# mobinasri/flagger

Measured on AMD Instinct MI355X. Metric: coverage windows/sec through EM+decode; achieved HBM GB/s vs roofline, higher is better.
Workload: dtype f64

## Files before the change

### flagger_amd/csrc/hf_create.h

```cpp
#pragma once

namespace {
struct PinnedArena {
    char *a = nullptr, *b = nullptr, *c = nullptr; std::thread th;
    ~PinnedArena() { if (th.joinable()) th.join(); pin_cache().release(a); pin_cache().release(b); pin_cache().release(c); }
};

struct KeyMarks {
    size_t words = 0;
    uint64_t gen = 0;
    std::atomic<int> claimed{0};
    std::vector<std::vector<uint16_t>> tabs;
    KeyMarks() : tabs(HF_PARTS + 8) {}
    uint16_t* mine() {
        static thread_local uint64_t tl_gen = 0;
        static thread_local int tl_slot = -1;
        if (tl_gen != gen) {
            tl_slot = claimed.fetch_add(1);
            tl_gen = gen;
            if (tl_slot < (int) tabs.size()) tabs[(size_t) tl_slot].assign(words, 0);
        }
        return tl_slot < (int) tabs.size() ? tabs[(size_t) tl_slot].data() : nullptr;
    }
};
// ... 382 lines not shown
        if (cw.ctrace) std::fprintf(stderr, "[hf_create] %d emission keys, %d (key, transition class) rows, %d slow windows\n",
                                    ctx->n_keys, n_combo, ctx->n_slow);
    }
    std::vector<SegDesc>& segs = ctx->h_segs;
    std::vector<int32_t>& cseg0 = cw.cseg0;
    cseg0.assign(C + 1, 0);
    int64_t nslots = 0;
    for (size_t c = 0; c < C; c++) {
        const int64_t t0 = w->chunk_off[c], T = w->chunk_off[c + 1] - t0;
        cseg0[c] = (int32_t) segs.size();
        if (T <= 0) continue;
        const int64_t nsg = (T + SMAX - 1) / SMAX, sz = (T + nsg - 1) / nsg;
        const int first = (int) segs.size();
        for (int64_t k = 0; k * sz < T; k++) {
            SegDesc d;
            std::memset(&d, 0, sizeof d);
            const int64_t w0 = k * sz, n = T - w0 < sz ? T - w0 : sz;
            d.t0 = t0 + w0; d.n = (int) n; d.L = (int) ((n + NL - 1) / NL);
            d.slot0 = (int32_t) nslots; nslots += (int64_t) d.L * NL;
            d.chunk_slow0 = ctx->n_combo + cw.soff[c];
            d.seg0 = first; d.k = (int) k; d.chunk = (int) c; d.ident_row = ctx->n_arows;
            d.reg_first = (int32_t) ((w->annot[t0] & 0xFC00000000000000ULL) >> 58);
            d.reg_last = (int32_t) ((w->annot[t0 + T - 1] & 0xFC00000000000000ULL) >> 58);
            segs.push_back(d);
        }
        const int nsc = (int) segs.size() - first;
        const int32_t spare = (int32_t) nslots++;
        for (int k = 0; k < nsc; k++) {
            segs[(size_t) (first + k)].nseg = nsc;
            segs[(size_t) (first + k)].next_slot = k + 1 < nsc ? segs[(size_t) (first + k + 1)].slot0 : spare;
        }
    }
    cseg0[C] = (int32_t) segs.size();
    ctx->h_cseg0 = cseg0;
    if (nslots < INT32_MAX) {
        ctx->nseg = (int) segs.size(); ctx->n_slots = nslots;
        CTRY(dev_upload(ctx, cw.stg, &ctx->d_chunk_seg0, cseg0.data(), cseg0.size()));
        CALLOC(ctx->d_seg_ready, segs.size() * 4);
        hipMemsetAsync(ctx->d_seg_ready, 0, segs.size() * 4, nullptr);
        CALLOC(ctx->d_seg_ll, segs.size() * 8);
        CALLOC(ctx->d_Pseg, segs.size() * 16 * 8);
    } else segs.clear();
    cw.phase("segments");
    return HF_OK;
}

struct StatsPlan {
    bool compact = false, planned = false;
    int64_t n_pos = 0;
    size_t np = 0;
    std::vector<int32_t> cnt;
    std::vector<int32_t> g_pos0;
    std::vector<int32_t> grp_ar, grp_n, grp_off;
    std::vector<RowSlot> rslots; std::vector<int32_t> rwreg, rwoff;
    std::vector<int64_t> extra0;
    std::vector<int32_t> h_spare;
};
int64_t plan_place_extras(CreateWork& cw, StatsPlan& pl, size_t sp, int64_t from, bool with_first_two) {
    hf_ctx* ctx = cw.ctx; const hf_windows* w = cw.w;
    int64_t p = from;
    const auto& sb = ctx->subs[sp];
    for (int c = sb.c0; c < sb.c1; c++) {
        const int64_t T = w->chunk_off[c + 1] - w->chunk_off[c];
        pl.extra0[(size_t) c] = p;
        p += T <= 0 ? 0 : (with_first_two ? (T < 2 ? T : 2) : 0) + 1;
        pl.extra0[(size_t) c + 1] = p;
    }
    for (int k = sb.seg0; k < sb.seg1; k++) ctx->h_segs[(size_t) k].trash_pos = (int32_t) p++;
    return p;
}

void plan_groups_and_slots(CreateWork& cw, StatsPlan& pl, int bpw) {
    hf_ctx* ctx = cw.ctx; const hf_windows* w = cw.w;
    const int n_regions = cw.n_regions;
    const size_t n_ar = cw.h_arow_src.size(), S = (size_t) cw.n_sub;
    const bool compact = pl.compact;
    std::vector<hf_ctx::SubPass>& subs = ctx->subs;
    struct Occ { int32_t region, ar; };
    std::vector<Occ> occ;
    const size_t MMr = (size_t) ctx->M * ctx->M;
    for (size_t r = 0; r < n_ar; r++) {
        bool any = false;
        for (size_t sp = 0; sp < S && !any; sp++) any = pl.cnt[sp * n_ar + r] != 0;
        if (!any) continue;
        const int64_t er = cw.h_arow_src[r];
        int32_t reg;
        if (er < ctx->n_lut) reg = (int32_t) ((size_t) er / MMr);
        else reg = (int32_t) ((w->annot[(size_t) cw.slow[(size_t) (er - ctx->n_lut)]] & 0xFC00000000000000ULL) >> 58);
        occ.push_back({reg, (int32_t) r});
    }
    if (n_regions > 1) std::stable_sort(occ.begin(), occ.end(), [](const Occ& a, const Occ& b) { return a.region < b.region; });
    const size_t nocc = occ.size();
    pl.g_pos0.assign(S * n_ar, 0);
    const size_t unit = (size_t) 16 * (size_t) bpw;
    struct RowBase { int32_t g0, slot0, go; int64_t p0; };
    std::vector<RowBase> rb(S * nocc, RowBase{0, 0, 0, 0});
    size_t n_grp = 0, n_slot = 0;
    int64_t next_pos = 0;
    for (size_t sp = 0; sp < S; sp++) {
        subs[sp].g0 = (int) n_grp; subs[sp].p0 = next_pos;
        for (size_t oi = 0; oi < nocc; oi++) {
            const size_t r = (size_t) occ[oi].ar;
            const int32_t c_ = pl.cnt[sp * n_ar + r];
            if (!c_) continue;
            RowBase& B = rb[sp * nocc + oi];
            B.g0 = (int32_t) n_grp;
            B.p0 = compact ? next_pos : subs[sp].p0 + (int64_t) (n_grp - (size_t) subs[sp].g0) * HF_GRP_PAIRS;
            n_grp += (size_t) ((c_ + HF_GRP_PAIRS - 1) / HF_GRP_PAIRS);
            if (compact) next_pos += c_;
        }
        if (!compact) next_pos = subs[sp].p0 + (int64_t) (n_grp - (size_t) subs[sp].g0) * HF_GRP_PAIRS;
        subs[sp].g1 = (int) n_grp;
        next_pos = plan_place_extras(cw, pl, sp, next_pos, true);
        subs[sp].p1 = next_pos;
    }
    pl.n_pos = next_pos;
    {
        size_t oi0 = 0;
        for (int reg = 0; reg < n_regions; reg++) {
            pl.rwoff[(size_t) reg] = (int32_t) (n_slot / unit);
            size_t oi1 = oi0;
            while (oi1 < nocc && occ[oi1].region == reg) oi1++;
            for (size_t sp = 0; sp < S; sp++) {
                int64_t open_row = -1; size_t run_slot0 = n_slot; int32_t run_groups = 0;
                for (size_t oi = oi0; oi < oi1; oi++) {
                    const size_t r = (size_t) occ[oi].ar;
                    const int32_t c_ = pl.cnt[sp * n_ar + r];
                    if (!c_) continue;
                    const int64_t er = cw.h_arow_src[r];
                    const int32_t ng = (c_ + HF_GRP_PAIRS - 1) / HF_GRP_PAIRS;
                    if (er != open_row) { n_slot = run_slot0 + (size_t) ((run_groups + HF_ROWSLOT_GROUPS - 1) / HF_ROWSLOT_GROUPS); run_slot0 = n_slot; run_groups = 0; open_row = er; }
                    rb[sp * nocc + oi].slot0 = (int32_t) run_slot0; rb[sp * nocc + oi].go = run_groups;
                    run_groups += ng;
                }
                n_slot = run_slot0 + (size_t) ((run_groups + HF_ROWSLOT_GROUPS - 1) / HF_ROWSLOT_GROUPS);
            }
            n_slot = (n_slot + HF_RS_WPB * unit - 1) / (HF_RS_WPB * unit) * (HF_RS_WPB * unit);
            for (size_t k = (size_t) pl.rwoff[(size_t) reg]; k < n_slot / unit; k++) pl.rwreg.push_back(reg);
            oi0 = oi1;
        }
    }
    pl.grp_ar.assign((n_grp + 3) / 4 * 4, 0); pl.grp_n.assign((n_grp + 3) / 4 * 4, 0);
    pl.grp_off.assign(n_grp + 1, 0);
    pl.rslots.assign(n_slot, RowSlot{-1, 0, 0, 0});
    for (size_t sp = 0; sp < S; sp++)
        for (size_t oi = 0; oi < nocc; oi++) {
            const size_t r = (size_t) occ[oi].ar;
            const int32_t c_ = pl.cnt[sp * n_ar + r];
            if (!c_) continue;
            const int64_t er = cw.h_arow_src[r];
            const RowBase B = rb[sp * nocc + oi];
            pl.g_pos0[sp * n_ar + r] = (int32_t) B.p0;
            int32_t xpx;
            if (er < ctx->n_lut) xpx = (int32_t) (((size_t) er / (size_t) ctx->M) % (size_t) ctx->M) | ((int32_t) ((size_t) er % (size_t) ctx->M) << 8);
            else { const size_t t = (size_t) cw.slow[(size_t) (er - ctx->n_lut)]; xpx = (int32_t) (w->cov[t] & 0xffu) | ((int32_t) (w->cov[t - 1] & 0xffu) << 8); }
            int64_t p = B.p0;
            for (int32_t j = 0, left = c_; left > 0; j++, left -= HF_GRP_PAIRS) {
                const size_t g = (size_t) (B.g0 + j);
                const int32_t here = left < HF_GRP_PAIRS ? left : HF_GRP_PAIRS;
                pl.grp_ar[g] = (int32_t) r; pl.grp_n[g] = here; pl.grp_off[g] = (int32_t) p;
                p += compact ? here : HF_GRP_PAIRS;
                RowSlot& sl = pl.rslots[(size_t) B.slot0 + (size_t) ((B.go + j) / HF_ROWSLOT_GROUPS)];
                if ((B.go + j) % HF_ROWSLOT_GROUPS == 0) { sl.row = (int32_t) er; sl.g0 = (int32_t) g; sl.ng = 1; sl.xpx = xpx; }
                else sl.ng++;
            }
        }
    pl.rwoff[(size_t) n_regions] = (int32_t) (pl.rslots.size() / unit);
    ctx->n_parts = 1;
    for (int reg = 0; reg < n_regions; reg++) if (pl.rwoff[(size_t) reg + 1] > pl.rwoff[(size_t) reg]) ctx->n_parts++;
    ctx->n_groups = (int) n_grp;
    pl.grp_off[n_grp] = (int32_t) (n_grp ? pl.grp_off[n_grp - 1] + (compact ? pl.grp_n[n_grp - 1] : HF_GRP_PAIRS) : 0);
    ctx->plan_compact = compact;
    pl.planned = true;
}

int plan_upload(CreateWork& cw, StatsPlan& pl) {
    hf_ctx* ctx = cw.ctx;
    const int n_regions = cw.n_regions;
    const size_t C = cw.C;
    {
        std::vector<int32_t> boff((size_t) n_regions * 256 + 1, 0), blist;
        auto bin_of = [&](size_t k) {
            const int x = pl.rslots[k].xpx & 0xff;
            return (size_t) pl.rwreg[k / ((size_t) 16 * (size_t) ctx->rs_bpw)] * 256 + (size_t) (x < HF_NB_MAX_COVERAGE ? x : HF_NB_MAX_COVERAGE - 1);
        };
        for (size_t k = 0; k < pl.rslots.size(); k++) if (pl.rslots[k].row >= 0) boff[bin_of(k) + 1]++;
        for (size_t b = 0; b + 1 < boff.size(); b++) boff[b + 1] += boff[b];
        blist.resize((size_t) boff.back());
        std::vector<int32_t> fill(boff.begin(), boff.end() - 1);
        for (size_t k = 0; k < pl.rslots.size(); k++) if (pl.rslots[k].row >= 0) blist[(size_t) fill[bin_of(k)]++] = (int32_t) k;
        CTRY(dev_upload(ctx, cw.stg, &ctx->d_bin_off, boff.data(), boff.size()));
        CTRY(dev_upload(ctx, cw.stg, &ctx->d_bin_list, blist.data(), blist.size()));
        CALLOC(ctx->d_slot_h, pl.rslots.size() * 4 * 8);
        CALLOC(ctx->d_H, (size_t) n_regions * 4 * 256 * 8);
    }
    ctx->n_rowwaves = (int) (pl.rslots.size() / ((size_t) 16 * (size_t) ctx->rs_bpw));
    CTRY(dev_upload(ctx, cw.stg, &ctx->d_grp_ar, pl.grp_ar.data(), pl.grp_ar.size()));
    CTRY(dev_upload(ctx, cw.stg, &ctx->d_grp_n, pl.grp_n.data(), pl.grp_n.size()));
    if (pl.compact) CTRY(dev_upload(ctx, cw.stg, &ctx->d_grp_off, pl.grp_off.data(), pl.grp_off.size()));
    CTRY(dev_upload(ctx, cw.stg, &ctx->d_rowslots, pl.rslots.data(), pl.rslots.size()));
    CTRY(dev_upload(ctx, cw.stg, &ctx->d_rw_region, pl.rwreg.data(), pl.rwreg.size()));
    CTRY(dev_upload(ctx, cw.stg, &ctx->d_rw_off, pl.rwoff.data(), pl.rwoff.size()));
    ctx->h_rw_off = pl.rwoff;
    CALLOC(ctx->d_grp_sums, (size_t) pl.grp_ar.size() * 16 * 8);
    CALLOC(ctx->d_chunk_ll, C * 8);
    CALLOC(ctx->d_rw_stats, (size_t) ctx->n_rowwaves * (16 + 9 + 2 + 3 * 16 + 1) * 8);
    ctx->rows_ready = true;
    return HF_OK;
}

int create_statistics_plan(CreateWork& cw) {
    hf_ctx* ctx = cw.ctx; const hf_windows* w = cw.w;
    const size_t N = cw.N, C = cw.C;
    const int n_regions = cw.n_regions;
    if (!(N > 0 && C > 0 && ctx->nseg > 0)) return HF_OK;
    const size_t n_ar = cw.h_arow_src.size();
    const size_t S = (size_t) cw.n_sub;
    StatsPlan pl;
    pl.cnt.assign(S * n_ar + 1, 0);
    pl.rwoff.assign((size_t) n_regions + 1, 0);
    pl.extra0.assign(C + 1, 0);
    pl.h_spare.assign(C, 0);
    for (size_t c = 0; c < C; c++) {
        const int64_t T = w->chunk_off[c + 1] - w->chunk_off[c];
        pl.np += (size_t) (T > 2 ? T - 2 : 0);
    }
    for (auto& h : cw.pcnt)
        if (!h.empty())
            for (size_t r = 0; r < S * n_ar; r++) { const int32_t here = h[r]; h[r] = pl.cnt[r]; pl.cnt[r] += here; }
    int64_t n_groups_all = 0;
    for (size_t r = 0; r < S * n_ar; r++) n_groups_all += (pl.cnt[r] + HF_GRP_PAIRS - 1) / HF_GRP_PAIRS;
    const bool dense = n_groups_all * HF_GRP_PAIRS <= 4 * (int64_t) pl.np + (4 << 20);
    pl.compact = !dense;
    const char* const force = std::getenv("HF_STATS_PLAN");
    if (force && std::strstr(force, "compact")) pl.compact = true;
    if (force && std::strstr(force, "padded") && n_groups_all * HF_GRP_PAIRS + 3 * (int64_t) C + 4 * HF_GRP_PAIRS < INT32_MAX) pl.compact = false;
    int bpw = 1;
    while (bpw < 8 && n_groups_all / 16 / (2 * bpw) >= 1000) bpw *= 2;
    if (force) { const char* b = std::strstr(force, "bpw="); if (b) { const int v = std::atoi(b + 4); if (v >= 1 && v <= 64) bpw = v; } }
    ctx->rs_bpw = bpw;
    cw.phase("plan: pairs");
    int32_t* const pos = cw.P2;
    if (w->chunk_off[0] != 0 || (size_t) w->chunk_off[C] != N) std::memset(pos, 0, N * 4);
    std::vector<hf_ctx::SubPass>& subs = ctx->subs;
    subs.assign(S, hf_ctx::SubPass{0, 0, 0, 0, 0, 0, 0, 0});
    for (size_t sp = 0; sp < S; sp++) { subs[sp].c0 = (int) C; subs[sp].c1 = 0; }
    for (size_t c = 0; c < C; c++) {
        hf_ctx::SubPass& sb = subs[(size_t) cw.sub_of[c]];
        if ((int) c < sb.c0) sb.c0 = (int) c;
        if ((int) c + 1 > sb.c1) sb.c1 = (int) c + 1;
    }
    for (size_t sp = 0; sp < S; sp++) {
// ... 229 lines not shown
```

### flagger_amd/csrc/hf_estep.hip

```cpp
#include "hf_device.h"
#include <hip/hip_ext.h>
#include "../../include/hmm_flagger_model.h"
#ifndef HF_SCAN_L
#define HF_SCAN_L 4
#endif
#include <string>
#include <algorithm>
#include <vector>
#include <cstring>
#include <cstdio>
#include <cmath>
#include <atomic>
#include <functional>
#include <condition_variable>
#include <mutex>
#include <memory>
#include <chrono>
#include <cstdlib>

#include <thread>
#include <immintrin.h>
static thread_local std::string g_err;

constexpr size_t HF_PARTS = 64;
// ... 194 lines not shown
    double* d_b = nullptr;
    std::vector<int64_t> h_off; std::vector<int32_t> h_tile0;
    double* d_scale = nullptr;
    int8_t* d_label = nullptr;
    double* d_chunk_stats = nullptr;
    bool own_chunk_stats = true;
    double* d_total = nullptr;
    double* d_total_host = nullptr;
    TileDesc* d_tile_desc = nullptr;
    int ntiles = 0; int32_t* d_chunk_tile0 = nullptr;
    bool host_trace = false; double ht[5] = {0, 0, 0, 0, 0}; long ht_n = 0;
    double* d_tile_ll = nullptr;
    double* d_tile_stats = nullptr;
    unsigned* d_flags = nullptr;
    TableJob* d_jobs = nullptr; TabWork tabwork{};
    DevParams* d_params = nullptr; DevParams* h_params = nullptr; size_t params_bytes = 0;
    KParams kparams{};
    bool kp_ok = true, kp_now = false;
    unsigned* h_flags = nullptr;
    int8_t* h_label = nullptr;
    int8_t* d_label_host = nullptr;
    double* h_total = nullptr;
    hipEvent_t ev0 = nullptr, ev1 = nullptr; bool ev_valid = false;
    double ksum[HF_NKERNELS] = {}; int64_t kcount[HF_NKERNELS] = {};
    float klast[HF_NKERNELS] = {}; bool klast_ok[HF_NKERNELS] = {};
    unsigned prof_mask = 0;
    int prof_stride = 1; long prof_pass = 0; bool prof_now = true;
    hipEvent_t kev[2 * HF_NKERNELS] = {}; bool kran[HF_NKERNELS] = {};
    bool have_full = false;
    size_t lds_max = 64 * 1024;
    bool launch_failed = false;
    double beta_star = 1.0;
    int M = 1; double* d_lutE = nullptr; double* d_lutC = nullptr; int64_t n_lut = 0;
    int n_keys = 0; int32_t* d_keys = nullptr;
    double *d_nbE = nullptr, *d_nbP = nullptr, *d_nbDig = nullptr, *d_nbR = nullptr, *d_nbBeta = nullptr, *d_tile_hist = nullptr;
    char* h_nb[2] = {nullptr, nullptr}; hipEvent_t nb_ev[2] = {nullptr, nullptr}; bool nb_ev_used[2] = {false, false}; unsigned nb_turn = 0;
    int stats_mode = HF_STATS_CHUNKS; bool rows_ready = false, pass_rows = false; int pass_kc = 0, pass_wpb = 4;
    double poll_seq = 0.0;
    double* h_part = nullptr; double* d_part_host = nullptr; size_t part_cap = 0; bool host_total_ok = true, pass_host_total = false; int pass_rw_blocks = 0;
    std::vector<int32_t> h_rw_off;
    double* d_rank_out = nullptr; double* d_rank_flag = nullptr;
    bool pass_bound = false;
    bool stream_stamp_ok = true; uint32_t stream_stamp = 0;
    bool pass_polled = false;
    unsigned* d_done = nullptr;
    unsigned long long* d_cks = nullptr;
    int poll_kind = 0;
    int n_groups = 0, n_rowwaves = 0, n_parts = 1;
    bool pass_nb = false;
    int32_t* d_bin_off = nullptr; int32_t* d_bin_list = nullptr; double* d_slot_h = nullptr; double* d_H = nullptr;
    double* d_chunk_ll = nullptr;
    double* d_recs = nullptr;
    bool fb_recs = false, pass_pairs_done = false;
    struct SubPass { int c0, c1, seg0, seg1, g0, g1; int64_t p0, p1; int b0 = 0, b1 = 0; };
    std::vector<SubPass> subs;
    double* d_recs_all = nullptr; bool recs_all = false;
    bool scales_all = false;
    int32_t* d_grp_off = nullptr;
    bool plan_compact = false;
    int rs_bpw = 1;
    int32_t* d_grp_ar = nullptr; int32_t* d_grp_n = nullptr; double* d_grp_sums = nullptr;
    int32_t* d_pos_f = nullptr;
    int32_t* d_slot_of = nullptr;
    int32_t* d_pos = nullptr; int64_t n_pos = 0;
    RowSlot* d_rowslots = nullptr; int32_t* d_rw_region = nullptr; int32_t* d_rw_off = nullptr; double* d_rw_stats = nullptr;
    SegDesc* d_seg = nullptr; int nseg = 0; int32_t* d_chunk_seg0 = nullptr; double* d_seg_ll = nullptr; double* d_Pseg = nullptr;
    double* d_segQ = nullptr;
    unsigned* d_seg_ready = nullptr; unsigned seg_epoch = 0; bool seg_fused = true, seg_test_timeout = false;
    int seg_nc = 0;
    int32_t* d_seg_of_block = nullptr; std::vector<int32_t> h_seg_of_block;
    hf_params last_p{}; int last_mode = HF_MODE_FULL;
    hipStream_t last_stream = nullptr;
    int32_t* d_arow = nullptr; int32_t* d_arow_src = nullptr; int32_t* d_arow_cls = nullptr; double* d_lutA = nullptr;
    int n_arows = 0, n_combo = 0;
    double* d_scale_s = nullptr; int64_t n_slots = 0;
    std::vector<SegDesc> h_segs;
    std::vector<int32_t> h_cseg0;
    std::vector<std::pair<const char*, double>> create_phases;
    bool pass_seg = false;
    unsigned long long* d_seg_trace = nullptr;
    int n_slow = 0; int64_t* d_slow_w = nullptr; int32_t* d_slow_off = nullptr; double* d_Es = nullptr; double* d_Cs = nullptr;
    struct Viterbi {
        DevParams* h_params = nullptr; DevParams* d_params = nullptr; double* d_nbE = nullptr;
        double2* d_rows = nullptr;
        uint8_t* d_bp = nullptr;
        int8_t* d_label = nullptr; double* d_ll = nullptr; int8_t* d_final = nullptr; unsigned* d_flags = nullptr;
        double* d_P = nullptr; int* d_PE = nullptr; double* d_S = nullptr; int* d_SE = nullptr;
        double* d_vin = nullptr; long long* d_vinE = nullptr;
        uint8_t* d_lmap = nullptr; uint8_t* d_smap = nullptr; uint8_t* d_sexit = nullptr;
        bool alloc = false, launched = false, done = false;
        std::vector<double> h_ll;
    } vit;
};

static int cseg0_of(const hf_ctx* ctx, int c) { return ctx->h_cseg0[(size_t) c]; }
static void* ctx_alloc(hf_ctx* ctx, size_t bytes) {
    bytes = (bytes ? bytes : 8);
    bytes = (bytes + 255) & ~(size_t) 255;
    if (bytes > ctx->slab_left) {
        const size_t want = std::max(bytes, ctx->slabs.empty() ? ctx->slab_first : (size_t) 64 << 20);
        char* p = nullptr;
        if (hipMalloc((void**) &p, want) != hipSuccess) {
            (void) hipGetLastError();
            if (want == bytes || hipMalloc((void**) &p, bytes) != hipSuccess) return nullptr;
            ctx->slabs.emplace_back(p, bytes);
            return p;
        }
        ctx->slabs.emplace_back(p, want);
        ctx->slab_cur = p; ctx->slab_left = want;
    }
    char* r = ctx->slab_cur;
// ... 128 lines not shown

struct TileGeom { unsigned blocks = 0, threads = 256; size_t lds = 0; bool ok = false; };
template <class Kern>
static TileGeom tile_geom(const hf_ctx* ctx, Kern kernel, size_t per_wave_bytes, bool with_tab = true, int wmax = 4) {
    TileGeom g;
    const size_t tab = with_tab ? (size_t) ctx->R * HF_TAB_STRIDE * 8 : 0;
    int w = wmax;
    while (w >= 1 && tab + (size_t) w * per_wave_bytes > ctx->lds_max) w--;
    if (w < 1) return g;
    g.threads = 64u * (unsigned) w;
    g.blocks = (unsigned) ((ctx->ntiles + w - 1) / w);
    g.lds = tab + (size_t) w * per_wave_bytes;
    g.ok = true;
    if (g.lds > 64 * 1024)
        g.ok = hipFuncSetAttribute(reinterpret_cast<const void*>(kernel), hipFuncAttributeMaxDynamicSharedMemorySize, (int) g.lds) == hipSuccess;
    return g;
}
#define TILE_GEOM_OR_FAIL(g) do { if (!(g).ok) { set_err(HF_E_ARG, "the per-region tables do not fit the LDS of one workgroup"); ctx->launch_failed = true; return; } } while (0)

static RowSrc row_src(const hf_ctx* ctx) {
    RowSrc S;
    S.lutE = ctx->d_lutE; S.lutC = ctx->d_lutC; S.Es = ctx->d_Es; S.Cs = ctx->d_Cs; S.M = ctx->M; S.K = ctx->K; S.n_lut = (int) ctx->n_lut;
    return S;
}

static const int32_t* ll_off(const hf_ctx* ctx) { return ctx->pass_seg ? ctx->d_chunk_seg0 : ctx->d_chunk_tile0; }
static const double* ll_part(const hf_ctx* ctx) { return ctx->pass_seg ? ctx->d_seg_ll : ctx->d_tile_ll; }

static bool seg_pass(const hf_ctx* ctx) { return ctx->algo == HF_ALGO_SCAN && ctx->nseg > 0; }

static bool rows_pass(const hf_ctx* ctx) { return ctx->stats_mode == HF_STATS_ROWS && ctx->rows_ready && ctx->algo == HF_ALGO_SCAN; }

static int poll_mode() {
    static const int mode = [] {
        const char* e = std::getenv("HF_POLL");
        if (!e) return 0;
        if (!std::strcmp(e, "debug")) return 2;
        return e[0] == '1' ? 1 : 0;
    }();
    return mode;
}
static bool poll_ok(const hf_ctx* ctx, int last_kernel) {
    return poll_mode() != 0 && ctx->d_total_host && !((ctx->prof_mask >> last_kernel) & 1u) && !(ctx->prof_mask & HF_PROF_PASS) &&
           !ctx->host_trace;
}
static double next_stamp(hf_ctx* ctx) { ctx->poll_seq += 1.0; ctx->h_total[ctx->V + 1] = 0.0; return ctx->poll_seq; }

static void launch_pair_sums(hf_ctx* ctx, hipStream_t st, const hf_ctx::SubPass& sb, const double* recs_eff) {
    const int n = sb.g1 - sb.g0;
    if (n <= 0) return;
    if (ctx->plan_compact)
        hipLaunchKernelGGL(k_pair_sums_compact, dim3((unsigned) ((n + 63) / 64)), dim3(256), 0, st, n, ctx->d_grp_ar + sb.g0, ctx->d_grp_off + sb.g0,
                           ctx->d_grp_n + sb.g0, ctx->d_lutA, recs_eff, ctx->d_grp_sums + (size_t) sb.g0 * 16);
    else
        hipLaunchKernelGGL(k_pair_sums, dim3((unsigned) ((n + 15) / 16)), dim3(256), 0, st, n, ctx->d_grp_ar + sb.g0, ctx->d_grp_n + sb.g0,
                           ctx->d_lutA, recs_eff + sb.p0 * 8, ctx->d_grp_sums + (size_t) sb.g0 * 16);
}

static void launch_seg_fb(hf_ctx* ctx, hipStream_t st, bool full, double* recs_eff, int sub, unsigned epoch, unsigned wait_epoch, bool timed, bool with_scales = true) {
    int g0 = sub >= 0 ? ctx->subs[(size_t) sub].seg0 : 0, n = sub >= 0 ? ctx->subs[(size_t) sub].seg1 - g0 : ctx->nseg;
    const int32_t* const sob = ctx->seg_fused ? ctx->d_seg_of_block : nullptr;
    if (sob) {
        g0 = sub >= 0 ? ctx->subs[(size_t) sub].b0 : 0;
        n = (sub >= 0 ? ctx->subs[(size_t) sub].b1 : ctx->subs.back().b1) - g0;
    }
    if (n <= 0) return;
    const int nc = ctx->seg_fused ? ctx->seg_nc : 0;
    const size_t lds = seg_lds_bytes(nc);
#define HF_SEG_FB_ARGS ctx->d_seg, ctx->d_arow, ctx->d_lutA, ctx->d_params, ctx->d_segQ, ctx->d_Pseg, ctx->d_seg_ready, epoch, wait_epoch, ctx->d_pos, recs_eff, \
                        with_scales ? ctx->d_scale_s : (double*) nullptr, ctx->d_label, ctx->d_seg_ll, ctx->d_flags, (int32_t) g0, nc, sob
#define HF_SEG_FB_LAUNCH(B, F, CA) do { \
        if (timed) hipExtLaunchKernelGGL(HIP_KERNEL_NAME(k_seg_fb<B, F, CA>), dim3((unsigned) n), dim3(64), (uint32_t) lds, st, \
                                         ctx->kev[2 * HF_K_SEG_FB], ctx->kev[2 * HF_K_SEG_FB + 1], 0, HF_SEG_FB_ARGS); \
        else hipLaunchKernelGGL(HIP_KERNEL_NAME(k_seg_fb<B, F, CA>), dim3((unsigned) n), dim3(64), lds, st, HF_SEG_FB_ARGS); } while (0)
    if (nc > 0) { if (full) HF_SEG_FB_LAUNCH(true, true, true); else HF_SEG_FB_LAUNCH(false, true, true); }
    else if (full) { if (ctx->seg_fused) HF_SEG_FB_LAUNCH(true, true, false); else HF_SEG_FB_LAUNCH(true, false, false); }
    else { if (ctx->seg_fused) HF_SEG_FB_LAUNCH(false, true, false); else HF_SEG_FB_LAUNCH(false, false, false); }
#undef HF_SEG_FB_LAUNCH
#undef HF_SEG_FB_ARGS
}

static int all_records_buffer(hf_ctx* ctx) {
    if (ctx->d_recs_all) return HF_OK;
    int64_t n_pos = 0;
    for (const auto& sb : ctx->subs) if (sb.p1 > n_pos) n_pos = sb.p1;
    HIPCHK(hipMalloc((void**) &ctx->d_recs_all, (size_t) (n_pos + 1) * 64));
    return HF_OK;
}

template <int KT>
static void launch_stats(hf_ctx* ctx, hipStream_t st, int full, int ncol) {
    ctx->pass_rows = false; ctx->pass_host_total = false;
    if (full && rows_pass(ctx)) {
        KTimer t(ctx, st, HF_K_ROW_STATS);
        constexpr size_t NA = 16 + 9 + 2 + 3 * KT + 1;
        const int want_wpb = ctx->rs_bpw > 1 ? 4 : HF_RS_WPB;
        TileGeom g = tile_geom(ctx, k_row_stats<KT>, NA * 8, false, want_wpb);
        TILE_GEOM_OR_FAIL(g);
        if ((int) g.threads != 64 * want_wpb) { set_err(HF_E_ARG, "k_row_stats: the block's partial sums do not fit the LDS"); ctx->launch_failed = true; return; }
        const int wpb = (int) g.threads / 64;
        const int n_rw_blocks = (ctx->n_rowwaves + wpb - 1) / wpb, n_ll_blocks = (ctx->C + wpb - 1) / wpb;
        const bool bound = ctx->d_rank_out != nullptr;
        const bool polled = !bound && poll_ok(ctx, HF_K_ROW_STATS);
        const double seq = polled ? next_stamp(ctx) : 0.0;
        ctx->pass_polled = polled; ctx->pass_bound = bound;
        bool host_total = !bound && !polled && ctx->host_total_ok && ctx->d_total_host != nullptr;
        if (host_total) {
            const size_t need = (size_t) n_rw_blocks * NA + (size_t) ctx->C + 1;
            if (need > ctx->part_cap) {
// ... 93 lines not shown
        void *d = nullptr, *h = nullptr;
        if (hipMalloc(&d, 8 << 20) == hipSuccess && hipHostMalloc(&h, 8 << 20) == hipSuccess) {
            (void) hipMemcpy(d, h, 8 << 20, hipMemcpyHostToDevice);
            (void) hipMemcpy(h, d, 8 << 20, hipMemcpyDeviceToHost);
            (void) hipMemset(d, 0, 64);
        }
        if (h) hipHostFree(h);
        if (d) hipFree(d);
        (void) hipGetLastError();
    }
    {
        PinCache& pc = pin_cache();
        char* a = pc.acquire((size_t) 4 * (2u << 20));
        char* b = pc.acquire((size_t) 12 * (2u << 20));
        char* c = pc.acquire((size_t) 8 << 20);
        char* d = pc.acquire((size_t) 64 << 10);
        pc.release(a); pc.release(b); pc.release(c); pc.release(d);
    }
    return HF_OK;
}

void hf_destroy(hf_ctx* ctx) {
#ifdef HF_KSTAMP
    if (ctx && std::getenv("HF_KSTAMP_FILE")) {
        unsigned long long h[64 * 4 + 1];
        hipSetDevice(ctx->device); hipDeviceSynchronize();
        if (hipMemcpyFromSymbol(h, HIP_SYMBOL(g_kstamp), sizeof(h)) == hipSuccess)
            if (FILE* fp = std::fopen(std::getenv("HF_KSTAMP_FILE"), "ab")) { std::fwrite(h, 8, 64 * 4 + 1, fp); std::fclose(fp); }
    }
#endif
    if (!ctx) return;
    hipSetDevice(ctx->device);
#ifdef HF_SEG_TRACE
    if (ctx->d_seg_trace) {
        hipDeviceSynchronize();
        std::vector<unsigned long long> h((size_t) ctx->nseg * HF_SEG_TRACE_N);
        hipMemcpy(h.data(), ctx->d_seg_trace, h.size() * 8, hipMemcpyDeviceToHost);
        if (FILE* fp = std::fopen(std::getenv("HF_SEG_TRACE_FILE"), "wb")) { std::fwrite(h.data(), 8, h.size(), fp); std::fclose(fp); }
        unsigned long long* null_p = nullptr;
        hipMemcpyToSymbol(HIP_SYMBOL(g_seg_trace), &null_p, sizeof(void*));
        ctx_free(ctx, ctx->d_seg_trace);
    }
#endif
    if (ctx->host_trace && ctx->ht_n)
        std::fprintf(stderr, "[hf host trace] %ld EM steps: parameter view (hfm_params: the negative-binomial tables) %.1f us, enqueue %.1f us, wait %.1f us, m-step %.1f us, gpu span (first launch .. reduction) %.1f us\n",
                     ctx->ht_n, ctx->ht[4] / ctx->ht_n, ctx->ht[0] / ctx->ht_n, ctx->ht[1] / ctx->ht_n, ctx->ht[2] / ctx->ht_n, ctx->ht[3] / ctx->ht_n);
    ctx_free(ctx, ctx->d_off); ctx_free(ctx, ctx->d_rec); ctx_free(ctx, ctx->d_beta); ctx_free(ctx, ctx->d_regmask); ctx_free(ctx, ctx->d_E);
    ctx_free(ctx, ctx->d_f); ctx_free(ctx, ctx->d_b); ctx_free(ctx, ctx->d_scale); ctx_free(ctx, ctx->d_label); if (ctx->own_chunk_stats) ctx_free(ctx, ctx->d_chunk_stats);
    ctx_free(ctx, ctx->d_total); ctx_free(ctx, ctx->d_flags); ctx_free(ctx, ctx->d_params);
    ctx_free(ctx, ctx->d_lutE); ctx_free(ctx, ctx->d_lutC); ctx_free(ctx, ctx->d_slow_w); ctx_free(ctx, ctx->d_slow_off); ctx_free(ctx, ctx->d_keys);
    ctx_free(ctx, ctx->d_nbE); ctx_free(ctx, ctx->d_tile_hist);
    for (int b = 0; b < 2; b++) { if (ctx->h_nb[b]) hipHostFree(ctx->h_nb[b]); if (ctx->nb_ev[b]) hipEventDestroy(ctx->nb_ev[b]); }
    ctx_free(ctx, ctx->d_tile_desc); ctx_free(ctx, ctx->d_chunk_tile0);
    ctx_free(ctx, ctx->d_done); ctx_free(ctx, ctx->d_cks); ctx_free(ctx, ctx->d_bin_off); ctx_free(ctx, ctx->d_bin_list); ctx_free(ctx, ctx->d_slot_h); ctx_free(ctx, ctx->d_H); if (ctx->d_recs_all != ctx->d_recs) ctx_free(ctx, ctx->d_recs_all); ctx_free(ctx, ctx->d_recs); ctx_free(ctx, ctx->d_chunk_ll); ctx_free(ctx, ctx->d_grp_ar); ctx_free(ctx, ctx->d_grp_n); ctx_free(ctx, ctx->d_grp_off); ctx_free(ctx, ctx->d_pos); ctx_free(ctx, ctx->d_pos_f); ctx_free(ctx, ctx->d_slot_of); ctx_free(ctx, ctx->d_grp_sums); ctx_free(ctx, ctx->d_rowslots); ctx_free(ctx, ctx->d_rw_region);
    ctx_free(ctx, ctx->d_seg_of_block); ctx_free(ctx, ctx->d_seg); ctx_free(ctx, ctx->d_chunk_seg0); ctx_free(ctx, ctx->d_seg_ll); ctx_free(ctx, ctx->d_Pseg); ctx_free(ctx, ctx->d_segQ); ctx_free(ctx, ctx->d_seg_ready); ctx_free(ctx, ctx->d_scale_s);
    ctx_free(ctx, ctx->d_jobs); ctx_free(ctx, ctx->d_arow); ctx_free(ctx, ctx->d_arow_src); ctx_free(ctx, ctx->d_arow_cls); ctx_free(ctx, ctx->d_lutA);
    ctx_free(ctx, ctx->d_rw_off); ctx_free(ctx, ctx->d_rw_stats);
    ctx_free(ctx, ctx->d_tile_ll); ctx_free(ctx, ctx->d_tile_stats);
    vit_free(ctx);
    if (ctx->h_part) hipHostFree(ctx->h_part);
    if (ctx->h_label) pin_cache().release(reinterpret_cast<char*>(ctx->h_label));
    if (ctx->ev0) hipEventDestroy(ctx->ev0);
    if (ctx->ev1) hipEventDestroy(ctx->ev1);
    for (int i = 0; i < 2 * HF_NKERNELS; i++) if (ctx->kev[i]) hipEventDestroy(ctx->kev[i]);
    for (auto& sl : ctx->slabs) hipFree(sl.first);
    if (ctx->h_total) { hipDeviceSynchronize(); pin_cache().release(reinterpret_cast<char*>(ctx->h_total)); }
    delete ctx;
}

static int pack_params(hf_ctx* ctx, const hf_params* p, DevParams* dst = nullptr) {
    if (p->n_regions != ctx->R) return set_err(HF_E_ARG, "hf_estep: n_regions differs from hf_create");
    for (int s = 0; s < 4; s++)
        if (p->ncomp[s] < 1 || p->ncomp[s] > ctx->K) return set_err(HF_E_ARG, "hf_estep: ncomp out of range");
    if (p->ncomp[1] != 1 || p->ncomp[2] != 1 || p->ncomp[0] != 1)
        return set_err(HF_E_ARG, "hf_estep: Err/Dup/Hap must have one component (hmm_flagger.c:180-182)");
    DevParams* h = dst ? dst : ctx->h_params;
    h->model_type = p->model_type; h->n_regions = p->n_regions;
    h->beta_star = ctx->beta_star;
    for (int s = 0; s < 4; s++) h->ncomp[s] = p->ncomp[s];
    for (int pre = 0; pre < 4; pre++)
        for (int s = 0; s < 4; s++) h->alpha[pre * 4 + s] = p->alpha[pre][s];
    for (int s = 0; s < 4; s++) {
        int nu = 0;
        for (int pre = 0; pre < 4; pre++) {
            const double a = p->alpha[pre][s];
            int u = -1;
            for (int k = 0; k < nu; k++) if (h->ualpha[s][k] == a) { u = k; break; }
            if (u < 0) { u = nu; h->ualpha[s][nu++] = a; }
            h->umap[pre * 4 + s] = u;
        }
        for (int k = nu; k < 4; k++) h->ualpha[s][k] = 0.0;
        h->nuniq[s] = nu;
    }
    {
        int n = 0;
        for (int st = 0; st < 4; st++) {
            const bool te = st == 0 && p->model_type == HF_MODEL_TRUNC_EXP_GAUSSIAN;
            const int nu = te ? 1 : h->nuniq[st], nc = te ? 1 : p->ncomp[st];
            for (int u = 0; u < 4; u++) h->item_base[st * 4 + u] = u < nu ? n + u * nc : n;
            for (int u = 0; u < nu; u++)
                for (int c = 0; c < nc; c++) { h->item_s[n] = (uint8_t) st; h->item_u[n] = (uint8_t) u; h->item_c[n] = (uint8_t) c; n++; }
        }
        h->n_items = n;
    }
    for (int r = 0; r < ctx->R; r++) {
        DevRegion* g = &h->reg[r];
        std::memcpy(g->trans, p->trans + (size_t) r * 25, sizeof(double) * 25);
// ... 986 lines not shown
```

### flagger_amd/csrc/hf_rows.h

```cpp
#pragma once
#include <type_traits>
#include "hf_scan.h"

#define HF_GRP_PAIRS 64
#define HF_ROWSLOT_GROUPS 4


template <int CTRL>
__device__ __forceinline__ double quad_perm_f64(double v) {
    const int lo = __builtin_amdgcn_update_dpp(0, __double2loint(v), CTRL, 0xf, 0xf, false);
    const int hi = __builtin_amdgcn_update_dpp(0, __double2hiint(v), CTRL, 0xf, 0xf, false);
    return __hiloint2double(hi, lo);
}

__global__ void __launch_bounds__(256) k_pair_sums(int n_groups, const int32_t* __restrict__ grp_ar, const int32_t* __restrict__ grp_n,
                                                   const double* __restrict__ lutA, const double* __restrict__ recs,
                                                   double* __restrict__ grp_sums) {
    KSTAMP(2);
    const int wave = (int) ((blockIdx.x * 256u + threadIdx.x) >> 6), lane = threadIdx.x & 63;
    const int g0 = wave * 4;
    if (g0 >= n_groups) return;
    const int ql = lane & 3, qd = lane >> 2;
    const int pi = ql & 1, si = ql >> 1;
    const double2* __restrict__ R2 = reinterpret_cast<const double2*>(recs) + (int64_t) g0 * HF_GRP_PAIRS * 4 + lane;
    int ng[4];
#pragma unroll
    for (int g = 0; g < 4; g++) ng[g] = g0 + g < n_groups ? grp_n[g0 + g] : 0;
#pragma unroll
    for (int g = 0; g < 4; g++) {
        double2 v[4];
#pragma unroll
        for (int j = 0; j < 4; j++) {
            const bool have = j * 16 + qd < ng[g];
            v[j] = have ? R2[(g * 4 + j) * 64] : make_double2(0.0, 0.0);
        }
        double acc[4] = {0.0, 0.0, 0.0, 0.0};
#pragma unroll
        for (int j = 0; j < 4; j++) {
            const double f0 = quad_perm_f64<0x44>(v[j].x), f1 = quad_perm_f64<0x44>(v[j].y);
            const double b0 = quad_perm_f64<0xFA>(v[j].x), b1 = quad_perm_f64<0xFA>(v[j].y);
            acc[0] += f0 * b0; acc[1] += f1 * b0; acc[2] += f0 * b1; acc[3] += f1 * b1;
        }
#pragma unroll
        for (int u = 0; u < 4; u++) {
            double x = acc[u];
            x += __shfl_xor(x, 4); x += __shfl_xor(x, 8); x += __shfl_xor(x, 16); x += __shfl_xor(x, 32);
            acc[u] = x;
        }
        if (qd == 0 && g0 + g < n_groups) {
            const double* __restrict__ A = lutA + (int64_t) grp_ar[g0 + g] * 16;
            double* __restrict__ dst = grp_sums + (int64_t) (g0 + g) * 16;
#pragma unroll
            for (int u = 0; u < 4; u++) {
                const int kk = HF_PS(2 * pi + (u & 1), 2 * si + (u >> 1));
                dst[kk] = acc[u] * A[kk];
            }
        }
    }
}

__global__ void __launch_bounds__(256) k_pair_sums_compact(int n_groups, const int32_t* __restrict__ grp_ar, const int32_t* __restrict__ grp_off,
                                                           const int32_t* __restrict__ grp_n,
                                                           const double* __restrict__ lutA, const double* __restrict__ recs,
                                                           double* __restrict__ grp_sums) {
    const int wave = (int) ((blockIdx.x * 256u + threadIdx.x) >> 6), lane = threadIdx.x & 63;
    const int ql = lane & 3, g = wave * 16 + (lane >> 2);
    const int pi = ql & 1, si = ql >> 1;
    int base = 0, n = 0;
    if (g < n_groups) { base = grp_off[g]; n = grp_n[g]; }
    const double2* __restrict__ R2 = reinterpret_cast<const double2*>(recs) + (int64_t) base * 4 + ql;
    double acc[4] = {0.0, 0.0, 0.0, 0.0};
    for (int k0 = 0; __any(k0 < n); k0 += 4) {
        double2 v[4];
#pragma unroll
        for (int j = 0; j < 4; j++) v[j] = k0 + j < n ? R2[(k0 + j) * 4] : make_double2(0.0, 0.0);
#pragma unroll
        for (int j = 0; j < 4; j++) {
            const double f0 = quad_perm_f64<0x44>(v[j].x), f1 = quad_perm_f64<0x44>(v[j].y);
            const double b0 = quad_perm_f64<0xFA>(v[j].x), b1 = quad_perm_f64<0xFA>(v[j].y);
            acc[0] += f0 * b0; acc[1] += f1 * b0; acc[2] += f0 * b1; acc[3] += f1 * b1;
        }
    }
    if (g < n_groups) {
        const double* __restrict__ A = lutA + (int64_t) grp_ar[g] * 16;
        double* __restrict__ dst = grp_sums + (int64_t) g * 16;
#pragma unroll
        for (int u = 0; u < 4; u += 2) {
            const int kk = HF_PS(2 * pi, 2 * si + (u >> 1));
            const double2 a = *reinterpret_cast<const double2*>(A + kk);
            *reinterpret_cast<double2*>(dst + kk) = make_double2(acc[u] * a.x, acc[u + 1] * a.y);
        }
    }
}

__device__ __forceinline__ void xcu_store(double* p, double v) { __hip_atomic_store(p, v, __ATOMIC_RELAXED, __HIP_MEMORY_SCOPE_SYSTEM); }
__device__ __forceinline__ double xcu_load(const double* p) { return __hip_atomic_load(p, __ATOMIC_RELAXED, __HIP_MEMORY_SCOPE_SYSTEM); }

#define HF_DONE_REGION0 1
#define HF_DONE_PARTS (HF_DONE_REGION0 + HF_MAXREGIONS + 1)
#define HF_DONE_WORDS (HF_DONE_PARTS + 1)
__host__ __device__ __forceinline__ double* done_scratch(unsigned* done) { return reinterpret_cast<double*>(done + ((HF_DONE_WORDS + 1) & ~1)); }
#define HF_DONE_BYTES ((((HF_DONE_WORDS + 1) & ~1) * 4) + (HF_MAXREGIONS + 1) * 8)

#ifndef HF_RS_WPB
#define HF_RS_WPB 8
#endif
static_assert(HF_RS_WPB % 4 == 0 && HF_RS_WPB <= 16, "regions are padded to whole blocks of HF_RS_WPB wavefronts; the negative-binomial kernels use 4");
#ifndef HF_ROWS_TOTAL_INFLIGHT
#define HF_ROWS_TOTAL_INFLIGHT 32
// ... 327 lines not shown
```

Measured before the change: 15.74 billion.

## Stream pair-sum groups per wave with cost-balanced plan and software-pipelined buffer loads

Replaces the fixed four-groups-per-wave mapping in k_pair_sums with a host-planned list of wave start groups. The plan packs a variable number of groups, up to 64, into each wave according to their record counts. Inside a wave, groups are processed in a software pipeline of depth HF_PS_DEPTH. It uses raw buffer loads with size-bounded resources, so out-of-range pairs read as zero without predicates, and buffer stores with an out-of-range offset to mask lanes. The aim is to overlap record loads with DPP-based reductions and balance work across waves, at the cost of an extra planning pass, a device array, and more register pressure.

```diff
diff --git a/flagger_amd/csrc/hf_create.h b/flagger_amd/csrc/hf_create.h
--- a/flagger_amd/csrc/hf_create.h
+++ b/flagger_amd/csrc/hf_create.h
@@ -458,6 +458,7 @@
     std::vector<int32_t> cnt;
     std::vector<int32_t> g_pos0;
     std::vector<int32_t> grp_ar, grp_n, grp_off;
+    std::vector<int32_t> ps_wave_g0;
     std::vector<RowSlot> rslots; std::vector<int32_t> rwreg, rwoff;
     std::vector<int64_t> extra0;
     std::vector<int32_t> h_spare;
@@ -474,6 +475,29 @@
     }
     for (int k = sb.seg0; k < sb.seg1; k++) ctx->h_segs[(size_t) k].trash_pos = (int32_t) p++;
     return p;
+}
+
+#ifndef HF_PS_WAVE_RECS
+#define HF_PS_WAVE_RECS 256
+#endif
+#ifndef HF_PS_GROUP_COST
+#define HF_PS_GROUP_COST 64
+#endif
+void plan_stream_waves(hf_ctx* ctx, StatsPlan& pl) {
+    std::vector<int32_t>& w0 = pl.ps_wave_g0;
+    w0.clear();
+    for (auto& sb : ctx->subs) {
+        sb.w0 = (int) w0.size();
+        int64_t cost = 0; int in_run = 0;
+        for (int g = sb.g0; g < sb.g1; g++) {
+            const int64_t c = (int64_t) pl.grp_n[(size_t) g] + HF_PS_GROUP_COST;
+            if (in_run > 0 && (in_run == 64 || cost + c > HF_PS_WAVE_RECS + HF_PS_GROUP_COST)) { cost = 0; in_run = 0; }
+            if (in_run == 0) w0.push_back(g);
+            cost += c; in_run++;
+        }
+        sb.w1 = (int) w0.size();
+    }
+    w0.push_back(ctx->subs.empty() ? 0 : ctx->subs.back().g1);
 }
 
 void plan_groups_and_slots(CreateWork& cw, StatsPlan& pl, int bpw) {
@@ -574,6 +598,7 @@
     pl.rwoff[(size_t) n_regions] = (int32_t) (pl.rslots.size() / unit);
     ctx->n_parts = 1;
     for (int reg = 0; reg < n_regions; reg++) if (pl.rwoff[(size_t) reg + 1] > pl.rwoff[(size_t) reg]) ctx->n_parts++;
+    if (!compact) plan_stream_waves(ctx, pl);
     ctx->n_groups = (int) n_grp;
     pl.grp_off[n_grp] = (int32_t) (n_grp ? pl.grp_off[n_grp - 1] + (compact ? pl.grp_n[n_grp - 1] : HF_GRP_PAIRS) : 0);
     ctx->plan_compact = compact;
@@ -604,6 +629,7 @@
     CTRY(dev_upload(ctx, cw.stg, &ctx->d_grp_ar, pl.grp_ar.data(), pl.grp_ar.size()));
     CTRY(dev_upload(ctx, cw.stg, &ctx->d_grp_n, pl.grp_n.data(), pl.grp_n.size()));
     if (pl.compact) CTRY(dev_upload(ctx, cw.stg, &ctx->d_grp_off, pl.grp_off.data(), pl.grp_off.size()));
+    else CTRY(dev_upload(ctx, cw.stg, &ctx->d_ps_wave_g0, pl.ps_wave_g0.data(), pl.ps_wave_g0.size()));
     CTRY(dev_upload(ctx, cw.stg, &ctx->d_rowslots, pl.rslots.data(), pl.rslots.size()));
     CTRY(dev_upload(ctx, cw.stg, &ctx->d_rw_region, pl.rwreg.data(), pl.rwreg.size()));
     CTRY(dev_upload(ctx, cw.stg, &ctx->d_rw_off, pl.rwoff.data(), pl.rwoff.size()));
diff --git a/flagger_amd/csrc/hf_estep.hip b/flagger_amd/csrc/hf_estep.hip
--- a/flagger_amd/csrc/hf_estep.hip
+++ b/flagger_amd/csrc/hf_estep.hip
@@ -270,11 +270,12 @@
     double* d_chunk_ll = nullptr;
     double* d_recs = nullptr;
     bool fb_recs = false, pass_pairs_done = false;
-    struct SubPass { int c0, c1, seg0, seg1, g0, g1; int64_t p0, p1; int b0 = 0, b1 = 0; };
+    struct SubPass { int c0, c1, seg0, seg1, g0, g1; int64_t p0, p1; int b0 = 0, b1 = 0; int w0 = 0, w1 = 0; };
     std::vector<SubPass> subs;
     double* d_recs_all = nullptr; bool recs_all = false;
     bool scales_all = false;
     int32_t* d_grp_off = nullptr;
+    int32_t* d_ps_wave_g0 = nullptr;
     bool plan_compact = false;
     int rs_bpw = 1;
     int32_t* d_grp_ar = nullptr; int32_t* d_grp_n = nullptr; double* d_grp_sums = nullptr;
@@ -509,9 +510,11 @@
     if (ctx->plan_compact)
         hipLaunchKernelGGL(k_pair_sums_compact, dim3((unsigned) ((n + 63) / 64)), dim3(256), 0, st, n, ctx->d_grp_ar + sb.g0, ctx->d_grp_off + sb.g0,
                            ctx->d_grp_n + sb.g0, ctx->d_lutA, recs_eff, ctx->d_grp_sums + (size_t) sb.g0 * 16);
-    else
-        hipLaunchKernelGGL(k_pair_sums, dim3((unsigned) ((n + 15) / 16)), dim3(256), 0, st, n, ctx->d_grp_ar + sb.g0, ctx->d_grp_n + sb.g0,
-                           ctx->d_lutA, recs_eff + sb.p0 * 8, ctx->d_grp_sums + (size_t) sb.g0 * 16);
+    else {
+        const int nw = sb.w1 - sb.w0;
+        hipLaunchKernelGGL(k_pair_sums, dim3((unsigned) ((nw + 3) / 4)), dim3(256), 0, st, nw, ctx->d_ps_wave_g0 + sb.w0, sb.g0,
+                           ctx->d_grp_ar + sb.g0, ctx->d_grp_n + sb.g0, ctx->d_lutA, recs_eff + sb.p0 * 8, ctx->d_grp_sums + (size_t) sb.g0 * 16);
+    }
 }
 
 static void launch_seg_fb(hf_ctx* ctx, hipStream_t st, bool full, double* recs_eff, int sub, unsigned epoch, unsigned wait_epoch, bool timed, bool with_scales = true) {
@@ -711,7 +714,7 @@
     ctx_free(ctx, ctx->d_nbE); ctx_free(ctx, ctx->d_tile_hist);
     for (int b = 0; b < 2; b++) { if (ctx->h_nb[b]) hipHostFree(ctx->h_nb[b]); if (ctx->nb_ev[b]) hipEventDestroy(ctx->nb_ev[b]); }
     ctx_free(ctx, ctx->d_tile_desc); ctx_free(ctx, ctx->d_chunk_tile0);
-    ctx_free(ctx, ctx->d_done); ctx_free(ctx, ctx->d_cks); ctx_free(ctx, ctx->d_bin_off); ctx_free(ctx, ctx->d_bin_list); ctx_free(ctx, ctx->d_slot_h); ctx_free(ctx, ctx->d_H); if (ctx->d_recs_all != ctx->d_recs) ctx_free(ctx, ctx->d_recs_all); ctx_free(ctx, ctx->d_recs); ctx_free(ctx, ctx->d_chunk_ll); ctx_free(ctx, ctx->d_grp_ar); ctx_free(ctx, ctx->d_grp_n); ctx_free(ctx, ctx->d_grp_off); ctx_free(ctx, ctx->d_pos); ctx_free(ctx, ctx->d_pos_f); ctx_free(ctx, ctx->d_slot_of); ctx_free(ctx, ctx->d_grp_sums); ctx_free(ctx, ctx->d_rowslots); ctx_free(ctx, ctx->d_rw_region);
+    ctx_free(ctx, ctx->d_done); ctx_free(ctx, ctx->d_cks); ctx_free(ctx, ctx->d_bin_off); ctx_free(ctx, ctx->d_bin_list); ctx_free(ctx, ctx->d_slot_h); ctx_free(ctx, ctx->d_H); if (ctx->d_recs_all != ctx->d_recs) ctx_free(ctx, ctx->d_recs_all); ctx_free(ctx, ctx->d_recs); ctx_free(ctx, ctx->d_chunk_ll); ctx_free(ctx, ctx->d_grp_ar); ctx_free(ctx, ctx->d_grp_n); ctx_free(ctx, ctx->d_grp_off); ctx_free(ctx, ctx->d_ps_wave_g0); ctx_free(ctx, ctx->d_pos); ctx_free(ctx, ctx->d_pos_f); ctx_free(ctx, ctx->d_slot_of); ctx_free(ctx, ctx->d_grp_sums); ctx_free(ctx, ctx->d_rowslots); ctx_free(ctx, ctx->d_rw_region);
     ctx_free(ctx, ctx->d_seg_of_block); ctx_free(ctx, ctx->d_seg); ctx_free(ctx, ctx->d_chunk_seg0); ctx_free(ctx, ctx->d_seg_ll); ctx_free(ctx, ctx->d_Pseg); ctx_free(ctx, ctx->d_segQ); ctx_free(ctx, ctx->d_seg_ready); ctx_free(ctx, ctx->d_scale_s);
     ctx_free(ctx, ctx->d_jobs); ctx_free(ctx, ctx->d_arow); ctx_free(ctx, ctx->d_arow_src); ctx_free(ctx, ctx->d_arow_cls); ctx_free(ctx, ctx->d_lutA);
     ctx_free(ctx, ctx->d_rw_off); ctx_free(ctx, ctx->d_rw_stats);
diff --git a/flagger_amd/csrc/hf_rows.h b/flagger_amd/csrc/hf_rows.h
--- a/flagger_amd/csrc/hf_rows.h
+++ b/flagger_amd/csrc/hf_rows.h
@@ -6,55 +6,87 @@
 #define HF_ROWSLOT_GROUPS 4
 
 
+#ifndef HF_PS_DEPTH
+#define HF_PS_DEPTH 2
+#endif
+static_assert(HF_PS_DEPTH >= 1 && HF_PS_DEPTH <= 4, "k_pair_sums keeps HF_PS_DEPTH groups of registers");
 template <int CTRL>
 __device__ __forceinline__ double quad_perm_f64(double v) {
     const int lo = __builtin_amdgcn_update_dpp(0, __double2loint(v), CTRL, 0xf, 0xf, false);
     const int hi = __builtin_amdgcn_update_dpp(0, __double2hiint(v), CTRL, 0xf, 0xf, false);
     return __hiloint2double(hi, lo);
 }
-
-__global__ void __launch_bounds__(256) k_pair_sums(int n_groups, const int32_t* __restrict__ grp_ar, const int32_t* __restrict__ grp_n,
+template <int CTRL>
+__device__ __forceinline__ double dpp_f64(double v) {
+    const int lo = __builtin_amdgcn_mov_dpp(__double2loint(v), CTRL, 0xf, 0xf, true);
+    const int hi = __builtin_amdgcn_mov_dpp(__double2hiint(v), CTRL, 0xf, 0xf, true);
+    return __hiloint2double(hi, lo);
+}
+__device__ __forceinline__ double quads_to_lanes03(double x) {
+    x += dpp_f64<0x104>(x);
+    x += dpp_f64<0x108>(x);
+    x += __shfl_xor(x, 16);
+    x += __shfl_xor(x, 32);
+    return x;
+}
+
+__device__ __forceinline__ __amdgpu_buffer_rsrc_t hf_buf(const void* base, int bytes) {
+    return __builtin_amdgcn_make_buffer_rsrc(const_cast<void*>(base), (short) 0, bytes, 0x00020000);
+}
+__device__ __forceinline__ double2 hf_u4_d2(const __attribute__((ext_vector_type(4))) unsigned v) {
+    return make_double2(__hiloint2double((int) v[1], (int) v[0]), __hiloint2double((int) v[3], (int) v[2]));
+}
+
+__global__ void __launch_bounds__(256) k_pair_sums(int n_waves, const int32_t* __restrict__ wave_g0, int g_base,
+                                                   const int32_t* __restrict__ grp_ar, const int32_t* __restrict__ grp_n,
                                                    const double* __restrict__ lutA, const double* __restrict__ recs,
                                                    double* __restrict__ grp_sums) {
     KSTAMP(2);
-    const int wave = (int) ((blockIdx.x * 256u + threadIdx.x) >> 6), lane = threadIdx.x & 63;
-    const int g0 = wave * 4;
-    if (g0 >= n_groups) return;
-    const int ql = lane & 3, qd = lane >> 2;
+    constexpr int D = HF_PS_DEPTH;
+    constexpr int OUT = 1 << 30;
+    const int wave = __builtin_amdgcn_readfirstlane((int) ((blockIdx.x * 256u + threadIdx.x) >> 6)), lane = threadIdx.x & 63;
+    if (wave >= n_waves) return;
+    const int g0 = wave_g0[wave] - g_base, ng = wave_g0[wave + 1] - g_base - g0;
+    const int ql = lane & 3;
     const int pi = ql & 1, si = ql >> 1;
-    const double2* __restrict__ R2 = reinterpret_cast<const double2*>(recs) + (int64_t) g0 * HF_GRP_PAIRS * 4 + lane;
-    int ng[4];
-#pragma unroll
-    for (int g = 0; g < 4; g++) ng[g] = g0 + g < n_groups ? grp_n[g0 + g] : 0;
-#pragma unroll
-    for (int g = 0; g < 4; g++) {
-        double2 v[4];
-#pragma unroll
-        for (int j = 0; j < 4; j++) {
-            const bool have = j * 16 + qd < ng[g];
-            v[j] = have ? R2[(g * 4 + j) * 64] : make_double2(0.0, 0.0);
-        }
-        double acc[4] = {0.0, 0.0, 0.0, 0.0};
-#pragma unroll
-        for (int j = 0; j < 4; j++) {
-            const double f0 = quad_perm_f64<0x44>(v[j].x), f1 = quad_perm_f64<0x44>(v[j].y);
-            const double b0 = quad_perm_f64<0xFA>(v[j].x), b1 = quad_perm_f64<0xFA>(v[j].y);
-            acc[0] += f0 * b0; acc[1] += f1 * b0; acc[2] += f0 * b1; acc[3] += f1 * b1;
-        }
-#pragma unroll
-        for (int u = 0; u < 4; u++) {
-            double x = acc[u];
-            x += __shfl_xor(x, 4); x += __shfl_xor(x, 8); x += __shfl_xor(x, 16); x += __shfl_xor(x, 32);
-            acc[u] = x;
-        }
-        if (qd == 0 && g0 + g < n_groups) {
-            const double* __restrict__ A = lutA + (int64_t) grp_ar[g0 + g] * 16;
-            double* __restrict__ dst = grp_sums + (int64_t) (g0 + g) * 16;
-#pragma unroll
-            for (int u = 0; u < 4; u++) {
-                const int kk = HF_PS(2 * pi + (u & 1), 2 * si + (u >> 1));
-                dst[kk] = acc[u] * A[kk];
-            }
+    const int my_n = lane < ng ? grp_n[g0 + lane] : 0;
+    const int my_ar = lane < ng ? grp_ar[g0 + lane] : 0;
+    const double* __restrict__ wrecs = recs + (int64_t) g0 * HF_GRP_PAIRS * 8;
+    const int kA = HF_PS(2 * pi, 2 * si);
+    const __amdgpu_buffer_rsrc_t out = hf_buf(grp_sums + (int64_t) g0 * 16, ng * 128);
+    double2 v[D][4], a[D][2];
+    auto issue = [&](int st, int k) {
+        const bool in = k < ng;
+        const int kk = in ? k : 0;
+        const int n = in ? __builtin_amdgcn_readlane(my_n, kk) : 0;
+        const __amdgpu_buffer_rsrc_t rr = hf_buf(wrecs + (int64_t) kk * HF_GRP_PAIRS * 8, n * 64);
+#pragma unroll
+        for (int j = 0; j < 4; j++) v[st][j] = hf_u4_d2(__builtin_amdgcn_raw_buffer_load_b128(rr, lane * 16 + j * 1024, 0, 0));
+        const double2* __restrict__ A2 = reinterpret_cast<const double2*>(lutA + (int64_t) __builtin_amdgcn_readlane(my_ar, kk) * 16 + kA);
+        a[st][0] = A2[0];
+        a[st][1] = A2[2];
+    };
+#pragma unroll
+    for (int st = 0; st < D - 1; st++) issue(st, st);
+    for (int k0 = 0; k0 < ng; k0 += D) {
+#pragma unroll
+        for (int st = 0; st < D; st++) {
+            const int k = k0 + st;
+            issue((st + D - 1) % D, k + D - 1);
+            __builtin_amdgcn_sched_barrier(0);
+            double acc[4] = {0.0, 0.0, 0.0, 0.0};
+#pragma unroll
+            for (int j = 0; j < 4; j++) {
+                const double f0 = dpp_f64<0x44>(v[st][j].x), f1 = dpp_f64<0x44>(v[st][j].y);
+                const double b0 = dpp_f64<0xFA>(v[st][j].x), b1 = dpp_f64<0xFA>(v[st][j].y);
+                acc[0] += f0 * b0; acc[1] += f1 * b0; acc[2] += f0 * b1; acc[3] += f1 * b1;
+            }
+#pragma unroll
+            for (int u = 0; u < 4; u++) acc[u] = quads_to_lanes03(acc[u]);
+            const int o = lane < 4 ? k * 128 + kA * 8 : OUT;
+            const double2 d0 = make_double2(acc[0] * a[st][0].x, acc[1] * a[st][0].y), d1 = make_double2(acc[2] * a[st][1].x, acc[3] * a[st][1].y);
+            __builtin_amdgcn_raw_buffer_store_b128(__builtin_bit_cast(__attribute__((ext_vector_type(4))) unsigned, d0), out, o, 0, 0);
+            __builtin_amdgcn_raw_buffer_store_b128(__builtin_bit_cast(__attribute__((ext_vector_type(4))) unsigned, d1), out, o + 32, 0, 0);
         }
     }
 }
```

Result: no change. 15.84 billion (median of 6 runs) (+0.7%).
